# rogosprojects/klogs

Hardware: AMD Instinct MI355X
Metric: filtered log GB/s (whole node) at 1/2/4/8 MI355X; % of HBM peak (higher is better)
Workload: dtype u8

## Files before the change

### klogs_amd/csrc/klf_engine.cpp

```cpp
#include <hip/hip_runtime.h>

#include <unistd.h>

#include <algorithm>
#include <atomic>
#include <cerrno>
#include <chrono>
#include <condition_variable>
#include <cstdio>
#include <cstdlib>
#include <cstring>
#include <deque>
#include <memory>
#include <mutex>
#include <string>
#include <thread>
#include <vector>

#include "../../include/klf.h"
#include "../../include/klf_debug.h"
#include "klf_copypool.hpp"
#include "klf_fieldval.hpp"
#include "klf_groupkey.hpp"
#include "klf_kernels.hpp"
// ... 1265 lines not shown
  klf_engine* e = p.e;
  const klf_filter* f = p.f;
  const RunKnobs& k = p.k;
  const bool general = p.mode == klf::CompiledSet::kGeneral, none = p.mode == klf::CompiledSet::kNone;
  memset(static_cast<void*>(&a), 0, sizeof(a));
  a.bytes = p.d_bytes; a.segs = e->d_segs.as<SegDesc>(); a.nsegs = p.nsegs; a.ntiles = (uint32_t)p.ntiles;
  a.tile_seg = e->d_tile_seg.as<uint32_t>();
  a.build_tiles = (!p.same_layout && attempt == 0) ? 1u : 0u;
  a.tindex_wide = (p.ntiles > klf::kScanSmallTiles || k.tindex_wide) ? 1u : 0u;
  a.since_sec = f->since.sec; a.since_nsec = f->since.nsec; a.tail = f->tail;
  since_digits(f->since.sec, f->since.nsec, a.since_dig);
  a.grep_mode = (uint32_t)p.mode; a.match_all = e->cs.also_all ? 1u : 0u;
  a.lit = e->d_lit.as<uint8_t>(); a.lit_words = e->d_lit.as<uint32_t>(); a.lit_len = (uint32_t)e->cs.literal.size();
  a.lit_anchor = e->cs.literal_anchor;
  a.lit_anchor_byte = e->cs.literal.empty() ? 0u : e->cs.literal[e->cs.literal_anchor];
  memcpy(static_cast<void*>(&a.pats), &e->dpats, sizeof(a.pats));
  a.tstat = e->d_tstat.as<klf::TileStat>(); a.tile_base = e->d_tile_base.as<uint64_t>(); a.bsum = e->d_bsum.as<uint64_t>();
  a.slots = p.wave_pool ? nullptr : e->d_slots.as<uint32_t>(); a.wave_pool = p.wave_pool ? 1u : 0u;
  a.pool = e->d_pool.as<uint32_t>(); a.pool_cap = e->pool_cap; a.pool_chunk = s.pool_chunk;
  a.counters = e->d_counters.as<uint32_t>(); a.segout = segout_of(e);
  a.wpre = e->d_wpre.as<uint64_t>(); a.wgrp = a.wpre + p.nsegs + 1;
  a.out = e->d_out.as<uint8_t>(); a.out_cap = e->d_out.p ? e->d_out.cap : 0;
  a.stage_times = (f->flags & KLF_FILTER_STAGE_TIMES) && p.evs ? 1u : 0u;
  if (p.need_cand) { a.cand = e->d_cand.as<uint64_t>(); a.cand_cap = e->cand_cap; }
  if (p.need_hits) {
    a.qhits = e->d_qhits.as<uint64_t>(); a.qhits_cap = p.qhits_cap; a.hslots = e->d_hslots.as<uint16_t>();
    a.hflat = e->d_hflat.as<uint64_t>(); a.hflat_cap = p.hflat_cap;
  }
  a.trec = e->d_trec.as<klf::TRec>(); a.kbase = e->d_kbase.as<uint64_t>();
  a.truns = p.want_truns ? e->d_truns.as<uint32_t>() : nullptr;
// ... 1754 lines not shown
  std::vector<uint32_t> kinds;
  for (uint32_t i = 0; i < n; ++i) {
    ps.emplace_back(pats[i].bytes, pats[i].bytes + pats[i].len);
    kinds.push_back(pats[i].kind);
  }
  klf::CompiledSet cs;
  std::string err;
  int code = KLF_OK;
  if (!klf::compile_set(ps, kinds, cs, err, code)) return code;
  if (info) {
    info[0] = cs.qf_on ? 1u : 0u;
    info[1] = cs.qf_q;
    info[2] = cs.qf_stride;
    info[3] = cs.qf_needles;
    info[4] = cs.qf_anc_on ? 0x100u | cs.qf_anc_byte : 0u;
  }
  if (cs.mode != klf::CompiledSet::kGeneral || !cs.qf_on) return klf_debug_match(pats, n, content, len, match);
  *match = (cs.also_all || klf::prefilter_match(cs, content, len, phase)) ? 1 : 0;
  return KLF_OK;
}

extern "C" int klf_debug_prefilter_hits(const klf_pattern* pats, uint32_t n, const uint8_t* sample, size_t slen,
                                        const uint8_t* data, size_t dlen, uint64_t* out, char* layout, size_t cap) {
  if ((n && !pats) || (slen && !sample) || (dlen && !data) || !out) return KLF_EINVAL;
  std::vector<std::vector<uint8_t>> ps;
  std::vector<uint32_t> kinds;
  for (uint32_t i = 0; i < n; ++i) {
    ps.emplace_back(pats[i].bytes, pats[i].bytes + pats[i].len);
    kinds.push_back(pats[i].kind);
  }
// ... 5 lines not shown
  if (slen) {
    klf::DataStats st;
    klf::data_stats(sample, slen, cs.qf_fold, st);
    klf::place_needles(cs, &st);
  }
  const klf::PrefilterHits h = klf::prefilter_hits(cs, data, dlen);
  out[0] = cs.qf_stride;
  out[1] = cs.qf_q;
  out[2] = cs.qf_k;
  out[3] = cs.qf_anc_on ? 0x100u | cs.qf_anc_byte : 0u;
  out[4] = h.probes;
  out[5] = h.bitmap_hits;
  out[6] = h.anchor_hits;
  out[7] = h.verified;
  out[8] = h.pair_pass;
  if (layout && cap) { strncpy(layout, cs.qf_layout.c_str(), cap - 1); layout[cap - 1] = 0; }
  return KLF_OK;
}

extern "C" int klf_debug_compile(const klf_pattern* pats, uint32_t n, uint32_t* mode, char* err, size_t err_cap) {
  if ((n && !pats) || !mode) return KLF_EINVAL;
  std::vector<std::vector<uint8_t>> ps;
  std::vector<uint32_t> kinds;
  for (uint32_t i = 0; i < n; ++i) {
    ps.emplace_back(pats[i].bytes, pats[i].bytes + pats[i].len);
    kinds.push_back(pats[i].kind);
  }
  klf::CompiledSet cs;
  std::string e;
  int code = KLF_OK;
// ... 26 lines not shown
```

### klogs_amd/csrc/klf_kernels.hip

```cpp
#include <hip/hip_ext.h>
#include <hip/hip_runtime.h>

#include <cstdio>
#include <cstdlib>
#include <cstring>
#include <type_traits>

#include "klf_fieldval.hpp"
#include "klf_groupkey.hpp"
#include "klf_kernels.hpp"
#include "klf_ts.hpp"

namespace klf {
namespace {

#ifndef KLF_TIMELINE
#define KLF_TIMELINE 0
#endif
__device__ uint32_t g_abl_waves;
#if KLF_TIMELINE
__device__ uint64_t g_timeline[300000 * 8];
__device__ uint32_t g_lb_rounds, g_lb_spins;
#define KLF_STAMP(tile, k) do { if (threadIdx.x == 0 && (tile) < 300000) g_timeline[(size_t)(tile) * 8 + (k)] = __builtin_amdgcn_s_memtime(); } while (0)
#else
// ... 770 lines not shown
  if (MODE == kScanLit) {
    if (tl.dense) __threadfence_block();
    wave_lds_sync();
    lit_grep(list, tl.nlines, s_tile, s_lit, a, c, anc, pat, n);
  }
  if (tl.dense) __threadfence_block();
  wave_lds_sync();
}

constexpr uint32_t kNoHit = 0xFFFFFFFFu;
template <int QS, int QK, int QQ>
struct QProbe {
  static constexpr bool kMidIdx = QQ == 3 && QK == 2;
  static constexpr bool K3 = QK == 3 || QK == (int)kQfTwoLevel;
  static constexpr bool TWO = QK == (int)kQfTwoLevel;
  static_assert(!TWO || QS == 4, "the two-level probe runs at stride 4");
  static_assert(QQ == 3 || QQ == 4, "3- or 4-byte grams");
  const uint32_t* s_qf;
  const uint8_t* s_tile;
  uint32_t fold;
  struct Hash {
    uint32_t h, p, m, a;
  };
  __device__ __forceinline__ Hash hash(uint32_t g) const {
    const uint32_t gf = g | fold;
    const uint32_t f = K3 ? gf ^ bfe_u32(gf, 13, 11) : gf;
    Hash r;
    r.h = mul_u24(f, 0x9E3779u);
    if (QQ == 4) r.h = mad_u24(gf >> 8, 0x7F4A7Du, r.h);
    r.p = K3 ? mul_hi_u24(f, 0xC2B2AEu) : 0u;
    r.m = K3 ? mul_u24(f, 0x5BD1E9u) : 0u;
    r.a = TWO ? (((r.h >> 21) << 2) + kQfPairWords * 4u)
          : kMidIdx ? ((r.h >> 16) & ((kQfWords - 1u) << 2)) : ((r.h >> (32 - kQfBucketBits)) << 2);
    return r;
  }
  __device__ __forceinline__ uint32_t word(const Hash& r) const {
    return *reinterpret_cast<const uint32_t*>(reinterpret_cast<const uint8_t*>(s_qf) + r.a);
  }
  __device__ __forceinline__ static uint32_t test(uint32_t w, const Hash& r) {
    uint32_t t = K3 ? (w >> ((r.m >> 24) & 31u)) & (w >> (r.p & 31u))
                    : shr_byte1(w, r.h) & (w >> ((r.h >> 16) & 31u));
    if (K3) t &= w >> ((r.h >> 16) & 31u);
    if (TWO) t &= shr_byte1(w, r.m);
    return t;
  }
  __device__ __forceinline__ uint32_t hbits(uint32_t g) const {
    const Hash r = hash(g);
    return test(word(r), r);
  }
  template <class F>
  __device__ __forceinline__ void chunk_grams(const ScanTile& c, uint32_t ch, F&& f) const {
    const uint32_t o0 = c.my0 + 16u * ch;
    const uint4 x = *reinterpret_cast<const uint4*>(s_tile + o0);
    if constexpr (QS == 6) {
      f(x.x, 0);
      f(__builtin_amdgcn_alignbyte(x.z, x.y, 2u), 6);
      f(x.w, 12);
      return;
    }
    const uint32_t w4 = QS < 4 ? reinterpret_cast<const uint32_t*>(s_tile)[(o0 >> 2) + 4] : 0u;
    const uint32_t w[5] = {x.x, x.y, x.z, x.w, w4};
#pragma unroll
    for (int d = 0; d < 4; ++d)
// ... 69 lines not shown
      uint32_t w[2 * kPer];
#pragma unroll
      for (int k = 0; k < 2 * kPer; ++k) r[k] = hash(g[k]);
#pragma unroll
      for (int k = 0; k < 2 * kPer; ++k) w[k] = word(r[k]);
      uint32_t acc_a = 0, acc_b = 0;
#pragma unroll
      for (int k = 0; k < 2 * kPer; ++k) {
        const uint32_t t = test(w[k], r[k]);
        if (k < kPer) acc_a |= t; else acc_b |= t;
      }
      chit |= ((acc_a & 1u) << ca) | ((acc_b & 1u) << cb);
    }
    return chit;
  }
  __device__ __forceinline__ uint32_t fast_chunks(const ScanTile& c) const {
    const uint32_t rot = ((uint32_t)c.lane >> 1) & 7u;
    uint32_t chit = 0;
#pragma unroll
    for (int v = 0; v < (ABL(c, 4) ? 0 : 8); ++v) {
      const uint32_t ch = ((uint32_t)v + rot) & 7u;
      uint32_t acc = 0;
      chunk_grams(c, ch, [&](uint32_t g, int) __attribute__((always_inline)) { acc |= hbits(g); });
      chit |= (acc & 1u) << ch;
    }
    return chit;
  }
  __device__ __forceinline__ void positions(const ScanTile& c, uint32_t chit, uint32_t (&hq)[4]) const {
    for (uint32_t m = chit; m; m &= m - 1u) {
      const uint32_t ch = (uint32_t)__builtin_ctz(m);
      uint32_t hm = 0;
      chunk_grams(c, ch, [&](uint32_t g, int pos) __attribute__((always_inline)) { hm |= (hbits(g) & 1u) << pos; });
      or_quad(hq, ch >> 1, clip_chunk(c, hm, ch) << ((ch & 1u) * 16u));
    }
  }
  __device__ __forceinline__ void run(const ScanTile& c, uint32_t* s_list, uint32_t nlines, uint32_t (&hq)[4],
                                      uint32_t& xh) const {
    if constexpr (TWO) {
      two_level(c, s_list, nlines, hq, xh);
    } else {
      const uint32_t chit = (QS == 4 || QS == 6) ? fast_pairs(c) : fast_chunks(c);
      if (__any(chit != 0)) positions(c, chit, hq);
    }
  }
};
__device__ __forceinline__ void anchored_hits(const DevPatterns& P, const uint8_t* s_tile, const ScanTile& c, uint32_t anc,
                                              uint32_t pat, uint32_t afold, uint32_t (&hq)[4]) {
  const uint32_t* s32 = reinterpret_cast<const uint32_t*>(s_tile);
  const uint32_t npre = P.qf_anc_n, fold = P.qf_fold;
  for (uint32_t cm = anc; cm; cm &= cm - 1u) {
    const uint32_t ch = (uint32_t)__builtin_ctz(cm);
    const uint4 x = lane_chunk(s_tile, c, ch);
    uint32_t am = 0;
    for (uint32_t e = clip_chunk(c, eq_mask16(afold ? or4(x, afold) : x, pat), ch); e; e &= e - 1u) {
// ... 190 lines not shown

    LineCounts n;
    if (ABL(c, 128)) {
    } else if (!tl.dense) {
      line_work<MODE, FUSE>(s_list, a, c, ev, tl, s_tile, s_lit, any.anc, pat, fz, tile == range_t0, s_frun_all[FUSE ? wv : 0],
                            s_fmap_all[FUSE ? wv : 0], n);
    } else if (tl.pool_ok && !abl) {
      if (FUSE && lane == 0) a.counters[kCtrFuseBad] = 1u;
      line_work<MODE, FUSE>(a.pool + tl.pool_base, a, c, ev, tl, s_tile, s_lit, any.anc, pat, fz, tile == range_t0,
                            s_frun_all[FUSE ? wv : 0], s_fmap_all[FUSE ? wv : 0], n);
    }

    uint32_t tile_hits = 0;
    if constexpr (GEN) {
      uint32_t hq[4] = {0u, 0u, 0u, 0u}, xh = kNoHit;
      const QProbe<QS, QK, QQ> probe{s_qf, s_tile, a.pats.qf_fold};
      probe.run(c, s_list, tl.nlines, hq, xh);
      if (ANC && __any(any.anc != 0)) anchored_hits(a.pats, s_tile, c, any.anc, pat, afold, hq);
      if (ABL(c, 8)) {
        asm volatile("" ::"v"(hq[0] | hq[1] | hq[2] | hq[3] | xh));
        hq[0] = hq[1] = hq[2] = hq[3] = 0;
        xh = kNoHit;
      }
      if (__any((hq[0] | hq[1] | hq[2] | hq[3]) != 0u || xh != kNoHit) && (!abl || (KLF_ABL & (65536 | 131072))))
        tile_hits = emit_hits(a, c, hq, xh);
    }

    TileTotals tt;
    tt.pq = packed_counts(n, tl.nlines);
    tt.defer = __any(n.defer != 0);
    tt.hit = LIT && __any(n.hits != 0);
// ... 655 lines not shown
      uint4 E = Eb[0];
#pragma unroll
      for (int i = 1; i < kVerifyEnt; ++i)
        if (j == i) E = Eb[i];
      entry(E);
    }
  }
}

__device__ void verify_hit(const RunArgs& a, uint32_t tile, uint32_t s, int32_t p, const VerifyQ& vq) {
  const DevPatterns& P = a.pats;
  const SegDesc sd = a.segs[s];
  const int64_t rel_lo = (int64_t)(tile - sd.tile0) * kTile;
  const uint32_t gs = gword(a.bytes + sd.base + rel_lo + p);
  const uint32_t g = (gs | P.qf_fold) & P.qf_mask;
  const uint32_t b = qf_bucket(g, P.qf_w24, P.qf_k);
  verify_hit_from(a, tile, s, sd, p, gs, P.qf_head[b], P.qf_head[b + 1], vq);
}

constexpr int kVerifyBatch = 4;
struct VerifyLds {
  uint32_t qn[4];
  uint64_t qbuf[4][kVerifyQ][2];
};
__device__ __forceinline__ void verify_body(RunArgs& a, uint32_t bid, uint32_t nb, VerifyLds& L) {
  auto& s_qn = L.qn;
  auto& s_qbuf = L.qbuf;
  if (a.counters[2] || a.counters[kCtrHitsOver]) return;
  const int lane = threadIdx.x & 63, wv = threadIdx.x >> 6;
  if (lane == 0) s_qn[wv] = 0;
  wave_lds_sync();
// ... 13 lines not shown
      tile[u] = (uint32_t)hf;
      pp[u] = (int32_t)((hf >> 32) & 0xFFFFu);
      sg[u] = (uint32_t)(hf >> 48);
      if (sg[u] == 0xFFFFu) sg[u] = a.tile_seg[tile[u]];
    }
#pragma unroll
    for (int u = 0; u < kVerifyBatch; ++u) sd[u] = a.segs[sg[u]];
    uint32_t gg[kVerifyBatch];
#pragma unroll
    for (int u = 0; u < kVerifyBatch; ++u) {
      const int64_t rel_lo = (int64_t)(tile[u] - sd[u].tile0) * kTile;
      gg[u] = gword(a.bytes + sd[u].base + rel_lo + pp[u]);
    }
#pragma unroll
    for (int u = 0; u < kVerifyBatch; ++u) {
      const uint32_t b = qf_bucket((gg[u] | P.qf_fold) & P.qf_mask, P.qf_w24, P.qf_k);
      e0[u] = P.qf_head[b];
      e1[u] = P.qf_head[b + 1];
    }
    KLF_VSTAMP(1);
#pragma unroll
    for (int u = 0; u < kVerifyBatch; ++u)
      if (i0 + (uint32_t)u * stride < nf) {
#if KLF_ABL & 16
        if (pp[u] == 0x7FFF) atomicOr(&a.counters[13], sg[u]);
        continue;
#endif
        verify_hit_from(a, tile[u], sg[u], sd[u], pp[u], gg[u], e0[u], e1[u], vq);
      }
  }
  const uint32_t nh = a.counters[kCtrHits] < a.qhits_cap ? a.counters[kCtrHits] : a.qhits_cap;
// ... 3040 lines not shown
hipError_t launch_scan(const RunArgs& a, hipStream_t st, int num_cus) {
  const int occ = scan_occupancy<MODE, QS, QK, QQ, QA, FUSE>();
  uint32_t grid = (uint32_t)(num_cus * occ);
  if (grid > a.ntiles) grid = a.ntiles;
  if (FUSE) grid = (a.fuse_nranges + kThreads / 64 - 1) / (kThreads / 64);
  if (t_scan_ev[0])
    hipExtLaunchKernelGGL((k_scan<MODE, QS, QK, QQ, QA, FUSE>), dim3(grid), dim3(kThreads), 0, st, t_scan_ev[0],
                          t_scan_ev[1], 0, a, a.tile_seg, a.segs);
  else
    hipLaunchKernelGGL((k_scan<MODE, QS, QK, QQ, QA, FUSE>), dim3(grid), dim3(kThreads), 0, st, a, a.tile_seg,
                       a.segs);
  return hipGetLastError();
}
template <int QS, int QQ>
hipError_t launch_gen_q(const RunArgs& a, hipStream_t st, int num_cus) {
  if constexpr (QS == 4)
    if (a.pats.qf_k == kQfTwoLevel)
      return launch_scan<kScanGen, 4, (int)kQfTwoLevel, QQ>(a, st, num_cus);
  if constexpr (QS == 8)
    if (a.pats.qf_anc_on)
      return a.pats.qf_k == 2 ? launch_scan<kScanGen, QS, 2, QQ, true>(a, st, num_cus)
                              : launch_scan<kScanGen, QS, 3, QQ, true>(a, st, num_cus);
  if (a.pats.qf_anc_on) return hipErrorInvalidValue;
  return a.pats.qf_k == 2 ? launch_scan<kScanGen, QS, 2, QQ>(a, st, num_cus)
                          : launch_scan<kScanGen, QS, 3, QQ>(a, st, num_cus);
}
template <int QS>
hipError_t launch_gen(const RunArgs& a, hipStream_t st, int num_cus) {
  if constexpr (QS == 1)
    return a.pats.qf_w24 ? hipErrorInvalidValue : launch_gen_q<1, 3>(a, st, num_cus);
  else
    return a.pats.qf_w24 ? launch_gen_q<QS, 4>(a, st, num_cus) : launch_gen_q<QS, 3>(a, st, num_cus);
}
// ... 402 lines not shown
```

### klogs_amd/csrc/klf_kernels.hpp

```cpp
#pragma once
#include <hip/hip_runtime.h>
#include <stdint.h>

namespace klf {

constexpr int kThreads = 256;
constexpr int kLaneBytes = 128;
constexpr int kTile = 64 * kLaneBytes;
constexpr int kHalo = 64;
constexpr int kMaxFusedLiteral = 256;
constexpr uint64_t kSegAlign = 256;
constexpr uint64_t kAllocSlack = kTile + kHalo + 1024;
constexpr uint32_t kPlenEscape = 16383;
constexpr int kCompactLines = 1024;
constexpr uint32_t kNumCounters = 64;
constexpr uint32_t kCtrPool = 4;
constexpr uint32_t kMatchChunk = 8192;

constexpr int kSlots = kTile / 32 + 2;
constexpr uint32_t kScanSmallTiles = 1u << 20;
constexpr int kSlotStride = (kSlots + 3) & ~3;
constexpr int kRecHead = 4;
constexpr uint32_t kScanGroup = 8;
constexpr int kRecStride = (kRecHead + kSlots + 31) & ~31;
// ... 24 lines not shown
constexpr uint32_t kCtrTailDone = 18;
constexpr uint32_t kCtrPlanDone = 26;
constexpr uint32_t kCtrVerified = 10;
constexpr uint32_t kCtrDense = 14;
constexpr uint32_t kCtrFuseBad = 24;
constexpr uint32_t kCtrOutShort = 22;
constexpr uint32_t kCtrPairsOver = 15;
constexpr uint32_t kQfRegex = 1u << 24;
constexpr uint32_t kQfLoose = 1u << 25;
constexpr uint32_t kQfAnchored = 1u << 26;
constexpr size_t kNfaMaxLds = 64 * 1024;
constexpr uint32_t kCarryBias = 256;
constexpr uint32_t kRxPreNone = 0xFFFFFFFFu;
constexpr uint32_t kQfTwoLevel = 5;
constexpr uint32_t kQfPairWords = 2048;
__host__ __device__ inline uint32_t qf_pair_word(uint32_t p) { return (p >> 5) & (kQfPairWords - 1u); }
__host__ __device__ inline bool qf_k3(uint32_t k) { return k == 3 || k == kQfTwoLevel; }
__host__ __device__ inline uint32_t qf_f(uint32_t g, uint32_t k) {
  const uint32_t g24 = g & 0xFFFFFFu;
  return qf_k3(k) ? g24 ^ (g24 >> 13) : g24;
}
__host__ __device__ inline uint32_t qf_hash(uint32_t g, uint32_t w24, uint32_t k) {
  const uint32_t hi = w24 ? (g >> 8) & 0xFFFFFFu : 0u;
  return qf_f(g, k) * 0x9E3779u + hi * 0x7F4A7Du;
}
__host__ __device__ inline uint32_t qf_word(uint32_t h) { return h >> (32 - kQfBucketBits); }
__host__ __device__ inline uint32_t qf_bucket(uint32_t g, uint32_t w24, uint32_t k) {
  if (w24 == 0 && k == 2) return (qf_hash(g, w24, k) >> 18) & (kQfWords - 1u);
  if (k == kQfTwoLevel) return qf_hash(g, w24, k) >> 21;
  return qf_word(qf_hash(g, w24, k));
}
__host__ __device__ inline uint32_t qf_bloom_word(uint32_t g, uint32_t w24, uint32_t k) {
  return (k == kQfTwoLevel ? kQfPairWords : 0u) + qf_bucket(g, w24, k);
}
__host__ __device__ inline uint32_t qf_bits(uint32_t g, uint32_t h, uint32_t k) {
  const uint32_t f = qf_f(g, k);
  const uint32_t m = f * 0x5BD1E9u;
  if (!qf_k3(k)) return (1u << ((h >> 8) & 31u)) | (1u << ((h >> 16) & 31u));
  const uint32_t p = (uint32_t)(((uint64_t)f * 0xC2B2AEu) >> 32);
  const uint32_t b3 = (1u << ((m >> 24) & 31u)) | (1u << (p & 31u)) | (1u << ((h >> 16) & 31u));
  return k == kQfTwoLevel ? b3 | (1u << ((m >> 8) & 31u)) : b3;
}
__host__ __device__ inline bool qf_pass(const uint32_t* bm, uint32_t gq, uint32_t w24, uint32_t k) {
  if (k == kQfTwoLevel && !((bm[qf_pair_word(gq & 0xFFFFu)] >> (gq & 31u)) & 1u)) return false;
  const uint32_t h = qf_hash(gq, w24, k), bits = qf_bits(gq, h, k);
  return (bm[qf_bloom_word(gq, w24, k)] & bits) == bits;
}
constexpr uint32_t kGramHistPairs = 256;
constexpr uint32_t kGramHistWords = kGramHistPairs + 65536;
constexpr uint64_t kGramHistSample = 64u << 10;
constexpr uint32_t kQfK2MaxGrams = 1536;
__host__ __device__ inline bool qf_sampled(uint64_t p, uint32_t S) {
  if (S == 6) {
    const uint32_t r = (uint32_t)(p & 15u);
    return r == 0 || r == 6 || r == 12;
  }
  return p % S == 0;
}
// ... 78 lines not shown
  uint32_t nsegs;
  uint32_t ntiles;
  uint32_t* tile_seg;
  uint32_t build_tiles;
  uint32_t tindex_wide;
  int64_t since_sec;
  int32_t since_nsec;
  uint32_t since_dig[6];
  int64_t tail;
  uint32_t grep_mode;
  uint32_t match_all;
  const uint8_t* lit;
  uint32_t lit_len;
  uint32_t lit_anchor;
  uint32_t lit_anchor_byte;
  const uint32_t* lit_words;
  DevPatterns pats;
  TileStat* tstat;
  uint32_t* slots;
  uint32_t* pool;
  uint64_t pool_cap;
  uint32_t wave_pool;
  uint32_t pool_chunk;
  uint64_t* tile_base;
  uint64_t* bsum;
  uint64_t* mpart;
  uint64_t* csum;
  uint32_t* cmap;
  uint64_t cmap_cap;
  uint32_t* cseg;
// ... 239 lines not shown
```

### klogs_amd/csrc/klf_patterns.cpp

```cpp
#include "klf_patterns.hpp"

#include <algorithm>
#include <chrono>
#include <bitset>
#include <cstdio>
#include <cstdlib>
#include <cstring>
#include <map>
#include <set>
#include <unordered_map>
#include <queue>
#include <thread>

#include "../../include/klf.h"
#include "klf_kernels.hpp"

namespace klf {
namespace {

using ByteSet = std::bitset<256>;

ByteSet range_set(int lo, int hi) {
  ByteSet s;
  if (hi < lo) return s;
// ... 1351 lines not shown
  }
  size_t cap = 64;
  uint32_t shift = 26;
  while (cap < 2 * grams.size()) cap <<= 1, --shift;
  std::vector<uint32_t> seen(cap, ~0u);
  double hit_share = 0;
  for (uint32_t g : grams) {
    uint32_t i = (g * 0x9E3779B1u) >> shift;
    while (seen[i] != ~0u && seen[i] != g) i = (i + 1) & (uint32_t)(cap - 1);
    if (seen[i] == g) continue;
    seen[i] = g;
    hit_share += gram_share(st, g, c.qf_q);
  }
  const double samples = qf_samples_per_tile(c.qf_stride);
  double hits = samples * std::min(1.0, hit_share);
  const double per_probe = c.qf_k == kQfTwoLevel ? 6.0 + (c.qf_q == 4 ? 1.0 : 0.0)
                                                 : 7.0 + (c.qf_q == 4 ? 3.0 : 0.0) + (c.qf_k == 3 ? 6.5 : 0.0);
  double cost = per_probe * samples / 64.0;
  if (c.qf_anc_on) {
    cost += 60.0;
    double pass = 0;
    for (size_t j = 0; j + 1 < c.qf_anc_pre.size(); j += 2)
      pass += c.qf_anc_pre[j + 1] == ~0u ? gram_share(st, c.qf_anc_pre[j], 4)
                                         : gram_share(st, c.qf_anc_pre[j] & 0xFFFFFFu, 3);
    hits += 8192.0 * std::min(1.0, pass);
  }
  return cost + 40.0 * hits;
}

void place_tables(CompiledSet& out, const DataStats* st);

}

void place_needles(CompiledSet& out, const DataStats* st) {
  std::vector<uint32_t> ac_next, ac_dict;
  std::vector<uint8_t> ac_accept;
  std::vector<int32_t> ac_out;
  std::vector<uint64_t> rx_b, rx_follow;
  std::vector<CompiledSet::NeedleSet> variants;
  std::vector<int32_t> user_map;
  ac_next.swap(out.ac_next);
  ac_dict.swap(out.ac_dict);
  ac_accept.swap(out.ac_accept);
  ac_out.swap(out.ac_out);
  rx_b.swap(out.rx_b);
  rx_follow.swap(out.rx_follow);
  variants.swap(out.qf_variants);
  user_map.swap(out.user_map);
  CompiledSet best;
  double best_cost = 0;
  bool have = false;
  std::vector<std::string> seen;
  for (uint32_t v = 0; v < variants.size(); ++v)
    for (int cand = 0; cand < 4; ++cand) {
      const int anchored = cand & 1;
      const uint32_t qmax = cand < 2 ? 4u : 3u;
      if (qmax == 3 && !(st && st->nbytes)) continue;
      if (const char* qv = getenv("KLF_QF_QMAX"))
        if (st && st->nbytes && (uint32_t)atoi(qv) != qmax) continue;
      CompiledSet c = out;
      const auto& ns = variants[v];
      c.qf_variant = v;
      c.qf_needle = ns.s;
      c.qf_nflags = ns.flags;
      c.qf_nrx = ns.rx;
      c.qf_needles = (uint32_t)ns.s.size();
      c.rx_pre = ns.rx_pre;
      choose_layout(c, st, anchored != 0, qmax);
      if (anchored && !c.qf_anc_on) continue;
      {
        const std::string key = std::to_string(v) + "/" + c.qf_layout;
        if (std::find(seen.begin(), seen.end(), key) != seen.end()) continue;
        seen.push_back(key);
      }
      const auto t0 = std::chrono::steady_clock::now();
      place_tables(c, st);
      const auto t1 = std::chrono::steady_clock::now();
      double cost;
      if (st && st->nbytes) {
        cost = layout_cost(c, *st);
      } else {
        cost = 1e6 * qf_samples_per_tile(c.qf_stride) / 8192.0 + (c.qf_anc_on ? c.qf_anc_share * 1e3 : 0.0);
      }
      char buf[64];
      snprintf(buf, sizeof buf, " k=%u [est %.0f VALU/tile]", c.qf_k, cost);
      c.qf_layout += buf;
      if (getenv("KLF_DIAG"))
        fprintf(stderr, "[klf] layout candidate (variant %u): %s (tables %.0f us, cost %.0f us)\n", v, c.qf_layout.c_str(),
                std::chrono::duration<double, std::micro>(t1 - t0).count(),
                std::chrono::duration<double, std::micro>(std::chrono::steady_clock::now() - t1).count());
      if (!have || cost < best_cost) {
        best = std::move(c);
        best_cost = cost;
        have = true;
      }
    }
  if (have) out = std::move(best);
  out.qf_variants.swap(variants);
  out.user_map.swap(user_map);
  out.ac_next.swap(ac_next);
  out.ac_dict.swap(ac_dict);
  out.ac_accept.swap(ac_accept);
  out.ac_out.swap(ac_out);
  out.rx_b.swap(rx_b);
  out.rx_follow.swap(rx_follow);
}

namespace {

void place_tables(CompiledSet& out, const DataStats* st) {
  const uint32_t q = out.qf_q, S = out.qf_stride;
  const bool hist = st && st->pair.size() >= 65536 && st->pair_tot > 0;
  const double nsample = st && st->nbytes ? (double)st->nbytes : 1.0;
  static const double pair_w = getenv("KLF_QF_PAIRW") ? atof(getenv("KLF_QF_PAIRW")) : 0.05;
  const bool loose = out.qf_fold != 0;
  out.qf_bitmap.assign(kQfWords, 0u);
  out.qf_head.clear();
  out.qf_ent.clear();
  out.qf_nbytes.clear();
  auto gram_at = [&](const std::string& s, uint32_t k) {
    uint32_t g = 0;
    for (uint32_t b = 0; b < q; ++b) g |= (uint32_t)(uint8_t)s[k + b] << (8 * b);
    return (g | out.qf_fold) & out.qf_mask;
  };
  uint8_t rank[256];
// ... 24 lines not shown
    uint32_t get(uint32_t g) const { return cnt[slot(g)]; }
    void add(uint32_t g) {
      const uint32_t i = slot(g);
      key[i] = g;
      ++cnt[i];
    }
  } used(out.qf_needle.size() * S + 1);
  std::vector<uint64_t> gcost;
  std::vector<std::pair<uint32_t, uint32_t>> bent;
  bent.reserve(out.qf_needle.size() * S);
  const size_t n = out.qf_needle.size();
  size_t nprobed = 0;
  for (size_t i = 0; i < n; ++i) nprobed += out.qf_nshort[i] ? 0 : 1;
  const char* two = getenv("KLF_QF_TWO");
  const bool two_ok = S == 4 && !out.qf_anc_on && !(two && !strcmp(two, "0"));
  out.qf_k = (two_ok && two && !strcmp(two, "force")) ? kQfTwoLevel
             : nprobed * S <= kQfK2MaxGrams ? 2u : two_ok ? kQfTwoLevel : 3u;
  const uint32_t w24 = q == 4 ? 24u : 0u;
  for (uint32_t i = 0; i < n; ++i) {
    const std::string& s = out.qf_needle[i];
    if (out.qf_nshort[i]) {
      const uint32_t k = out.qf_nanc[i], g = gram_at(s, k);
      bent.push_back({qf_bucket(g, w24, out.qf_k), i << 8 | k});
      continue;
    }
    const uint32_t amax = (uint32_t)std::min<size_t>(s.size() - (q + S - 1), 255 - (S - 1));
    gcost.resize(amax + S);
    for (uint32_t k = 0; k < amax + S; ++k) {
      const uint32_t g = gram_at(s, k);
      const uint64_t u = used.get(g);
      uint64_t c;
      if (hist) {
// ... 5 lines not shown
        c = 2 * u;
        for (uint32_t b = 0; b < q; ++b) c += common((uint8_t)s[k + b]);
      }
      gcost[k] = c;
    }
    uint32_t best_a = 0;
    uint64_t best = UINT64_MAX;
    for (uint32_t a = 0; a <= amax; ++a) {
      uint64_t sc = 0;
      for (uint32_t j = 0; j < S; ++j) sc = hist ? sc + gcost[a + j] : std::max(sc, gcost[a + j]);
      if (sc < best) { best = sc; best_a = a; }
    }
    for (uint32_t j = 0; j < S; ++j) {
      const uint32_t k = best_a + j, g = gram_at(s, k);
      used.add(g);
      const uint32_t h = qf_hash(g, w24, out.qf_k);
      const uint32_t bw = qf_bucket(g, w24, out.qf_k);
      out.qf_bitmap[qf_bloom_word(g, w24, out.qf_k)] |= qf_bits(g, h, out.qf_k);
      if (out.qf_k == kQfTwoLevel) {
        const uint32_t g16 = g & 0xFFFFu, fv = out.qf_fold & 0xFFFFu & g16;
        for (uint32_t x = fv;; x = (x - 1u) & fv) {
          const uint32_t pr = g16 & ~x;
          out.qf_bitmap[qf_pair_word(pr)] |= 1u << (pr & 31u);
          if (!x) break;
        }
      }
      bent.push_back({bw, i << 8 | k});
    }
  }
  std::vector<uint32_t> noff;
  for (auto& ns : out.qf_needle) {
    noff.push_back((uint32_t)out.qf_nbytes.size());
    for (size_t b = 0; b < ns.size(); b += 4) {
      uint32_t w = 0;
      for (size_t j = 0; j < 4 && b + j < ns.size(); ++j) w |= (uint32_t)(uint8_t)ns[b + j] << (8 * j);
      out.qf_nbytes.push_back(w);
    }
  }
  out.qf_head.assign(kQfWords + 1, 0u);
  for (auto& be : bent) out.qf_head[be.first + 1]++;
  for (uint32_t b = 0; b < kQfWords; ++b) out.qf_head[b + 1] += out.qf_head[b];
  out.qf_ent.assign((size_t)bent.size() * 4, 0u);
  std::vector<uint32_t> fill(out.qf_head.begin(), out.qf_head.end() - 1);
  for (auto& be : bent) {
    const uint32_t v = be.second, i = v >> 8;
    uint32_t* en = &out.qf_ent[(size_t)fill[be.first]++ * 4];
    en[0] = noff[i];
    en[1] = (uint32_t)out.qf_needle[i].size() | (v & 0xFFu) << 16 | out.qf_nflags[i] |
            (out.qf_nshort[i] ? kQfAnchored : 0u);
    en[2] = out.qf_nrx[i];
    {
      const auto& nd = out.qf_needle[i];
      const uint32_t k = v & 0xFFu;
      uint32_t w = 0;
      for (uint32_t j = 0; j < 4 && k + j < nd.size(); ++j) w |= (uint32_t)(uint8_t)nd[k + j] << (8 * j);
      en[3] = w;
    }
  }
}

}

void stats_finish(DataStats& st) {
  st.marg.assign(256, 0.0);
  st.inv_marg.assign(256, 0.0);
  st.pair_tot = 0;
  st.inv_tot = 0;
  if (st.pair.size() >= 65536) {
    for (uint32_t x = 0; x < 65536; ++x) st.marg[x & 0xFFu] += st.pair[x];
    for (double m : st.marg) st.pair_tot += m;
    if (st.pair_tot > 0) {
      st.inv_tot = 1.0 / st.pair_tot;
      for (int c = 0; c < 256; ++c) st.inv_marg[c] = st.pair_tot / (st.marg[c] + 128.0);
// ... 27 lines not shown
    st.pair[g >> 16] += 2;
  }
  stats_finish(st);
}

PrefilterHits prefilter_hits(const CompiledSet& cs, const uint8_t* s, size_t n) {
  PrefilterHits r;
  const uint32_t S = cs.qf_stride, w24 = cs.qf_q == 4 ? 24u : 0u;
  for (size_t p = 0; p < n; ++p) {
    uint32_t g = 0;
    for (uint32_t b = 0; b < 4; ++b) g |= (uint32_t)(p + b < n ? s[p + b] : 0) << (8 * b);
    bool hit = false;
    if (qf_sampled(p, S)) {
      ++r.probes;
      const uint32_t gq = (g | cs.qf_fold) & cs.qf_mask;
      hit = qf_pass(cs.qf_bitmap.data(), gq, w24, cs.qf_k);
      r.bitmap_hits += hit;
      if (cs.qf_k == kQfTwoLevel) r.pair_pass += (cs.qf_bitmap[qf_pair_word(gq & 0xFFFFu)] >> (gq & 31u)) & 1u;
    }
    if (!hit && cs.qf_anc_on && ((uint32_t)s[p] | (cs.qf_anc_fold & 0xFFu)) == cs.qf_anc_byte) {
      for (size_t j = 0; j + 1 < cs.qf_anc_pre.size() && !hit; j += 2)
        hit = ((g | cs.qf_fold) & cs.qf_anc_pre[j + 1]) == cs.qf_anc_pre[j];
      r.anchor_hits += hit;
    }
    if (!hit) continue;
    const uint32_t b = qf_bucket((g | cs.qf_fold) & cs.qf_mask, w24, cs.qf_k);
    for (uint32_t e = cs.qf_head[b]; e < cs.qf_head[b + 1]; ++e) {
      const uint32_t* E = cs.qf_ent.data() + 4 * (size_t)e;
      const uint32_t m = E[1] & 0xFFFFu, k = (E[1] >> 16) & 0xFFu;
      const int64_t x = (int64_t)p - (int64_t)k;
      if (x < 0 || (uint64_t)x + m > n) continue;
      const uint8_t* nb = reinterpret_cast<const uint8_t*>(cs.qf_nbytes.data() + E[0]);
      const uint8_t lm = (E[1] & kQfLoose) ? 0x20 : 0;
      bool eq = true;
      for (uint32_t j = 0; j < m && eq; ++j) eq = (uint8_t)(s[x + j] | lm) == nb[j];
      r.verified += eq;
    }
  }
  return r;
}

// ... 9 lines not shown
    for (uint64_t m = c; m; m &= m - 1) nd |= cs.rx_follow[(size_t)r * 64 + __builtin_ctzll(m)];
    d = nd;
    if (!d) return false;
  }
  return (d & cs.rx_end[r]) != 0;
}

bool prefilter_match(const CompiledSet& cs, const uint8_t* s, size_t n, uint32_t phase) {
  const uint32_t S = cs.qf_stride;
  for (size_t p = 0; p < n; ++p) {
    uint32_t g = 0;
    for (uint32_t b = 0; b < 4; ++b) g |= (uint32_t)(p + b < n ? s[p + b] : 0) << (8 * b);
    bool hit = false;
    if (qf_sampled(p + 16 - phase % 16, S)) {
      const uint32_t gq = (g | cs.qf_fold) & cs.qf_mask;
      hit = qf_pass(cs.qf_bitmap.data(), gq, cs.qf_q == 4 ? 24u : 0u, cs.qf_k);
    }
    if (!hit && cs.qf_anc_on && ((uint32_t)s[p] | (cs.qf_anc_fold & 0xFFu)) == cs.qf_anc_byte)
      for (size_t j = 0; j + 1 < cs.qf_anc_pre.size() && !hit; j += 2)
        hit = ((g | cs.qf_fold) & cs.qf_anc_pre[j + 1]) == cs.qf_anc_pre[j];
    if (!hit) continue;
    g = (g | cs.qf_fold) & cs.qf_mask;
    const uint32_t b = qf_bucket(g, cs.qf_q == 4 ? 24u : 0u, cs.qf_k);
    for (uint32_t e = cs.qf_head[b]; e < cs.qf_head[b + 1]; ++e) {
      const uint32_t* E = cs.qf_ent.data() + 4 * (size_t)e;
      const uint32_t m = E[1] & 0xFFFFu, k = (E[1] >> 16) & 0xFFu;
      const int64_t x = (int64_t)p - (int64_t)k;
      if (x < 0 || (uint64_t)x + m > n) continue;
      const uint8_t* nb = reinterpret_cast<const uint8_t*>(cs.qf_nbytes.data() + E[0]);
      const uint8_t lm = (E[1] & kQfLoose) ? 0x20 : 0;
      bool eq = true;
      for (uint32_t j = 0; j < m && eq; ++j) eq = (uint8_t)(s[x + j] | lm) == nb[j];
      if (!eq) continue;
      if (!(E[1] & kQfRegex)) return true;
      if ((cs.rx_flags[E[2]] & 1u) || nfa_window(cs, E[2], s, n, (size_t)x)) return true;
    }
  }
  return false;
// ... 4 lines not shown
```

### klogs_amd/csrc/klf_patterns.hpp

```cpp
#pragma once
#include <stdint.h>
#include <stddef.h>

#include <array>
#include <string>
#include <vector>

namespace klf {

constexpr int kMaxRegexPositions = 64;
constexpr int kMaxRegexes = 1024;

struct GlushkovTables {
  std::vector<uint64_t> follow;
  uint64_t first = 0;
  uint64_t last = 0;
  uint64_t init0 = 0;
  uint64_t end_accept = 0;
  bool accept_at_start = false;
  bool accept_empty = false;
  std::vector<std::vector<uint8_t>> pos_bytes;
  std::vector<std::array<uint64_t, 4>> pos_bits;
  int npos = 0;
};
// ... 40 lines not shown
  uint32_t rx_classes = 0;
  std::vector<uint8_t> rx_class;
  std::vector<uint64_t> rx_b;
  std::vector<uint64_t> rx_follow;
  std::vector<uint64_t> rx_first, rx_last, rx_init0, rx_end;
  std::vector<uint32_t> rx_flags;
  std::vector<uint32_t> rx_pre;
  uint32_t rx_maxpos = 0;

  bool qf_on = false;
  uint32_t qf_q = 4;
  uint32_t qf_stride = 1;
  uint32_t qf_fold = 0;
  uint32_t qf_mask = ~0u;
  uint32_t qf_k = 3;
  std::vector<uint32_t> qf_bitmap;
  std::vector<uint32_t> qf_head;
  std::vector<uint32_t> qf_ent;
  std::vector<uint32_t> qf_nbytes;
  uint32_t qf_needles = 0;
  std::vector<std::string> qf_needle;
  std::vector<uint32_t> qf_nflags, qf_nrx;
  bool qf_tuned = false;
  std::string qf_why;
  bool qf_anc_on = false;
  uint32_t qf_anc_byte = 0;
  uint32_t qf_anc_fold = 0;
  double qf_anc_share = 0;
  std::vector<uint32_t> qf_anc_pre;
  std::vector<uint8_t> qf_nshort;
// ... 54 lines not shown
```

### klogs_amd/engine.py

```python
from __future__ import annotations

import ctypes as C
import os
from dataclasses import dataclass
from pathlib import Path
from typing import Iterable, List, Optional, Sequence, Tuple

import numpy as np

_LIB_DIR = Path(os.environ.get("KLF_LIB_DIR", Path(__file__).resolve().parent / "_lib"))
_LIB_PATH = _LIB_DIR / "libklf.so"

KLF_OK = 0
KLF_EINVAL = -1
KLF_ENOMEM = -2
KLF_EHIP = -3
KLF_EPATTERN = -4
KLF_ETOOBIG = -5
KLF_ESTATE = -6
KLF_EIO = -7
KLF_PAT_LITERAL = 0
KLF_PAT_REGEX = 1
GO_ZERO_TIME = (-62135596800, 0)
TIME_MIN_SEC = -(1 << 63)
# ... 266 lines not shown
    rc = _lib.klf_debug_compile(arr, n, C.byref(mode), err, 512)
    return rc, MODE_NAMES.get(mode.value, "?"), err.value.decode()


def debug_match(content: bytes, grep=(), match=()) -> bool:
    arr, n, keep = _patterns(grep, match)
    m = C.c_int()
    buf = C.create_string_buffer(content, len(content) or 1)
    _check(_lib.klf_debug_match(arr, n, buf, len(content), C.byref(m)))
    return bool(m.value)


def debug_prefilter(content: bytes, grep=(), match=(), phase: int = 0):
    arr, n, keep = _patterns(grep, match)
    m = C.c_int()
    info = (C.c_uint32 * 5)()
    buf = C.create_string_buffer(content, len(content) or 1)
    _check(_lib.klf_debug_prefilter(arr, n, buf, len(content), phase, C.byref(m), info))
    return bool(m.value), dict(on=bool(info[0]), q=info[1], stride=info[2], needles=info[3],
                               anchor=(info[4] & 0xFF) if info[4] else None)


def debug_prefilter_hits(sample: bytes, data: bytes, grep=(), match=()):
    arr, n, keep = _patterns(grep, match)
    out = (C.c_uint64 * 9)()
    lay = C.create_string_buffer(256)
    sb = C.create_string_buffer(sample, len(sample) or 1)
    db = C.create_string_buffer(data, len(data) or 1)
    _check(_lib.klf_debug_prefilter_hits(arr, n, sb, len(sample), db, len(data), out, lay, 256))
    return dict(stride=out[0], q=out[1], k=out[2], anchor=(out[3] & 0xFF) if out[3] else None, probes=out[4],
                bitmap_hits=out[5], anchor_hits=out[6], verified=out[7], pair_pass=out[8],
                layout=lay.value.decode())


def debug_factors(pattern: bytes, want: int = 0):
    buf = C.create_string_buffer(4096)
    n, pre, loose = C.c_uint32(), C.c_uint32(), C.c_uint32()
    p = C.create_string_buffer(pattern, len(pattern) or 1)
    rc = _lib.klf_debug_factors(p, len(pattern), want, buf, 4096, C.byref(n), C.byref(pre), C.byref(loose))
    if rc == KLF_EINVAL:
        return None
    _check(rc)
    alts = buf.raw.split(b"\0")[: n.value]
    return alts, (None if pre.value == 0xFFFFFFFF else pre.value), bool(loose.value)


# ... 444 lines not shown
```

Measured before the change: 5701.

## Add exact perfect-hash gram prefilter for small stride-4 needle sets

Adds a new prefilter mode (k=6) for small stride-4, unanchored needle sets. Grams are placed into a collision-free multiplicative-hash table that stores the full gram, so each probe is one LDS load and one compare instead of a Bloom test over several hash bits. The intent is fewer VALU operations per probe and fewer false-positive hits reaching verification. The layout chooser costs this candidate and selects it when sample stats are present. It adds host-side search for a collision-free multiplier and a new kernel instantiation, and falls back when more than 192 distinct grams exist or no multiplier is found.

After: 5861 (median of 6 runs). 1.03x the previous value.

```diff
diff --git a/klogs_amd/csrc/klf_engine.cpp b/klogs_amd/csrc/klf_engine.cpp
--- a/klogs_amd/csrc/klf_engine.cpp
+++ b/klogs_amd/csrc/klf_engine.cpp
@@ -1303,6 +1303,7 @@
   a.lit = e->d_lit.as<uint8_t>(); a.lit_words = e->d_lit.as<uint32_t>(); a.lit_len = (uint32_t)e->cs.literal.size();
   a.lit_anchor = e->cs.literal_anchor;
   a.lit_anchor_byte = e->cs.literal.empty() ? 0u : e->cs.literal[e->cs.literal_anchor];
+  a.qf_mul = e->cs.qf_mul;
   memcpy(static_cast<void*>(&a.pats), &e->dpats, sizeof(a.pats));
   a.tstat = e->d_tstat.as<klf::TileStat>(); a.tile_base = e->d_tile_base.as<uint64_t>(); a.bsum = e->d_bsum.as<uint64_t>();
   a.slots = p.wave_pool ? nullptr : e->d_slots.as<uint32_t>(); a.wave_pool = p.wave_pool ? 1u : 0u;
@@ -3087,6 +3088,8 @@
     info[2] = cs.qf_stride;
     info[3] = cs.qf_needles;
     info[4] = cs.qf_anc_on ? 0x100u | cs.qf_anc_byte : 0u;
+    info[5] = cs.qf_k;
+    info[6] = cs.qf_mul;
   }
   if (cs.mode != klf::CompiledSet::kGeneral || !cs.qf_on) return klf_debug_match(pats, n, content, len, match);
   *match = (cs.also_all || klf::prefilter_match(cs, content, len, phase)) ? 1 : 0;
@@ -3122,6 +3125,8 @@
   out[6] = h.anchor_hits;
   out[7] = h.verified;
   out[8] = h.pair_pass;
+  out[9] = cs.qf_grams;
+  out[10] = cs.qf_mul;
   if (layout && cap) { strncpy(layout, cs.qf_layout.c_str(), cap - 1); layout[cap - 1] = 0; }
   return KLF_OK;
 }
diff --git a/klogs_amd/csrc/klf_kernels.hip b/klogs_amd/csrc/klf_kernels.hip
--- a/klogs_amd/csrc/klf_kernels.hip
+++ b/klogs_amd/csrc/klf_kernels.hip
@@ -808,11 +808,14 @@
   static constexpr bool kMidIdx = QQ == 3 && QK == 2;
   static constexpr bool K3 = QK == 3 || QK == (int)kQfTwoLevel;
   static constexpr bool TWO = QK == (int)kQfTwoLevel;
+  static constexpr bool EX = QK == (int)kQfExact;
   static_assert(!TWO || QS == 4, "the two-level probe runs at stride 4");
+  static_assert(!EX || QS == 4, "the exact probe runs at stride 4");
   static_assert(QQ == 3 || QQ == 4, "3- or 4-byte grams");
   const uint32_t* s_qf;
   const uint8_t* s_tile;
   uint32_t fold;
+  uint32_t mul;
   struct Hash {
     uint32_t h, p, m, a;
   };
@@ -838,9 +841,19 @@
     if (TWO) t &= shr_byte1(w, r.m);
     return t;
   }
+  __device__ __forceinline__ uint32_t ex_sample(uint32_t g) const { return g | fold; }
+  __device__ __forceinline__ uint32_t ex_word(uint32_t gf) const {
+    const uint32_t a = (mul_u24(gf, mul) >> 16) & ((kQfWords - 1u) << 2);
+    return *reinterpret_cast<const uint32_t*>(reinterpret_cast<const uint8_t*>(s_qf) + a);
+  }
   __device__ __forceinline__ uint32_t hbits(uint32_t g) const {
-    const Hash r = hash(g);
-    return test(word(r), r);
+    if constexpr (EX) {
+      const uint32_t gf = ex_sample(g);
+      return ex_word(gf) == gf ? 1u : 0u;
+    } else {
+      const Hash r = hash(g);
+      return test(word(r), r);
+    }
   }
   template <class F>
   __device__ __forceinline__ void chunk_grams(const ScanTile& c, uint32_t ch, F&& f) const {
@@ -940,6 +953,24 @@
     }
     return chit;
   }
+  __device__ __forceinline__ uint64_t fast_exact(const ScanTile& c) const {
+    const uint32_t rot = ((uint32_t)c.lane >> 1) & 7u;
+    uint64_t lanes = 0;
+#pragma unroll
+    for (int v = 0; v < (ABL(c, 4) ? 0 : 8); v += 2) {
+      const uint4 xa = lane_chunk(s_tile, c, ((uint32_t)v + rot) & 7u);
+      const uint4 xb = lane_chunk(s_tile, c, ((uint32_t)v + 1u + rot) & 7u);
+      const uint32_t g[8] = {xa.x, xa.y, xa.z, xa.w, xb.x, xb.y, xb.z, xb.w};
+      uint32_t gf[8], w[8];
+#pragma unroll
+      for (int k = 0; k < 8; ++k) gf[k] = ex_sample(g[k]);
+#pragma unroll
+      for (int k = 0; k < 8; ++k) w[k] = ex_word(gf[k]);
+#pragma unroll
+      for (int k = 0; k < 8; ++k) lanes |= __ballot(w[k] == gf[k]);
+    }
+    return lanes;
+  }
   __device__ __forceinline__ uint32_t fast_chunks(const ScanTile& c) const {
     const uint32_t rot = ((uint32_t)c.lane >> 1) & 7u;
     uint32_t chit = 0;
@@ -964,6 +995,9 @@
                                       uint32_t& xh) const {
     if constexpr (TWO) {
       two_level(c, s_list, nlines, hq, xh);
+    } else if constexpr (EX) {
+      const uint64_t lanes = fast_exact(c);
+      if (lanes) positions(c, ((lanes >> c.lane) & 1u) ? 0xFFu : 0u, hq);
     } else {
       const uint32_t chit = (QS == 4 || QS == 6) ? fast_pairs(c) : fast_chunks(c);
       if (__any(chit != 0)) positions(c, chit, hq);
@@ -1184,7 +1218,9 @@
     uint32_t tile_hits = 0;
     if constexpr (GEN) {
       uint32_t hq[4] = {0u, 0u, 0u, 0u}, xh = kNoHit;
-      const QProbe<QS, QK, QQ> probe{s_qf, s_tile, a.pats.qf_fold};
+      constexpr bool EX = QK == (int)kQfExact;
+      const QProbe<QS, QK, QQ> probe{s_qf, s_tile, a.pats.qf_fold | ((EX && QQ == 3) ? 0xFF000000u : 0u),
+                                     EX ? a.qf_mul : 0u};
       probe.run(c, s_list, tl.nlines, hq, xh);
       if (ANC && __any(any.anc != 0)) anchored_hits(a.pats, s_tile, c, any.anc, pat, afold, hq);
       if (ABL(c, 8)) {
@@ -1870,7 +1906,7 @@
   const int64_t rel_lo = (int64_t)(tile - sd.tile0) * kTile;
   const uint32_t gs = gword(a.bytes + sd.base + rel_lo + p);
   const uint32_t g = (gs | P.qf_fold) & P.qf_mask;
-  const uint32_t b = qf_bucket(g, P.qf_w24, P.qf_k);
+  const uint32_t b = qf_bucket(g, P.qf_w24, P.qf_k, a.qf_mul);
   verify_hit_from(a, tile, s, sd, p, gs, P.qf_head[b], P.qf_head[b + 1], vq);
 }
 
@@ -1914,7 +1950,7 @@
     }
 #pragma unroll
     for (int u = 0; u < kVerifyBatch; ++u) {
-      const uint32_t b = qf_bucket((gg[u] | P.qf_fold) & P.qf_mask, P.qf_w24, P.qf_k);
+      const uint32_t b = qf_bucket((gg[u] | P.qf_fold) & P.qf_mask, P.qf_w24, P.qf_k, a.qf_mul);
       e0[u] = P.qf_head[b];
       e1[u] = P.qf_head[b + 1];
     }
@@ -4985,9 +5021,13 @@
 }
 template <int QS, int QQ>
 hipError_t launch_gen_q(const RunArgs& a, hipStream_t st, int num_cus) {
-  if constexpr (QS == 4)
+  if constexpr (QS == 4) {
     if (a.pats.qf_k == kQfTwoLevel)
       return launch_scan<kScanGen, 4, (int)kQfTwoLevel, QQ>(a, st, num_cus);
+    if (a.pats.qf_k == kQfExact && !a.pats.qf_anc_on)
+      return launch_scan<kScanGen, 4, (int)kQfExact, QQ>(a, st, num_cus);
+  }
+  if (a.pats.qf_k == kQfExact) return hipErrorInvalidValue;
   if constexpr (QS == 8)
     if (a.pats.qf_anc_on)
       return a.pats.qf_k == 2 ? launch_scan<kScanGen, QS, 2, QQ, true>(a, st, num_cus)
diff --git a/klogs_amd/csrc/klf_kernels.hpp b/klogs_amd/csrc/klf_kernels.hpp
--- a/klogs_amd/csrc/klf_kernels.hpp
+++ b/klogs_amd/csrc/klf_kernels.hpp
@@ -62,6 +62,13 @@
 constexpr uint32_t kRxPreNone = 0xFFFFFFFFu;
 constexpr uint32_t kQfTwoLevel = 5;
 constexpr uint32_t kQfPairWords = 2048;
+constexpr uint32_t kQfExact = 6;
+constexpr uint32_t kQfExactMaxGrams = 192;
+constexpr uint32_t kQfExactTries = 512;
+__host__ __device__ inline uint32_t qf_exact_slot(uint32_t g, uint32_t mul) {
+  return (((g & 0xFFFFFFu) * mul) >> 18) & (kQfWords - 1u);
+}
+__host__ __device__ inline uint32_t qf_exact_word(uint32_t g, uint32_t w24) { return w24 ? g : g | 0xFF000000u; }
 __host__ __device__ inline uint32_t qf_pair_word(uint32_t p) { return (p >> 5) & (kQfPairWords - 1u); }
 __host__ __device__ inline bool qf_k3(uint32_t k) { return k == 3 || k == kQfTwoLevel; }
 __host__ __device__ inline uint32_t qf_f(uint32_t g, uint32_t k) {
@@ -73,7 +80,8 @@
   return qf_f(g, k) * 0x9E3779u + hi * 0x7F4A7Du;
 }
 __host__ __device__ inline uint32_t qf_word(uint32_t h) { return h >> (32 - kQfBucketBits); }
-__host__ __device__ inline uint32_t qf_bucket(uint32_t g, uint32_t w24, uint32_t k) {
+__host__ __device__ inline uint32_t qf_bucket(uint32_t g, uint32_t w24, uint32_t k, uint32_t mul = 0u) {
+  if (k == kQfExact) return qf_exact_slot(g, mul);
   if (w24 == 0 && k == 2) return (qf_hash(g, w24, k) >> 18) & (kQfWords - 1u);
   if (k == kQfTwoLevel) return qf_hash(g, w24, k) >> 21;
   return qf_word(qf_hash(g, w24, k));
@@ -89,7 +97,8 @@
   const uint32_t b3 = (1u << ((m >> 24) & 31u)) | (1u << (p & 31u)) | (1u << ((h >> 16) & 31u));
   return k == kQfTwoLevel ? b3 | (1u << ((m >> 8) & 31u)) : b3;
 }
-__host__ __device__ inline bool qf_pass(const uint32_t* bm, uint32_t gq, uint32_t w24, uint32_t k) {
+__host__ __device__ inline bool qf_pass(const uint32_t* bm, uint32_t gq, uint32_t w24, uint32_t k, uint32_t mul = 0u) {
+  if (k == kQfExact) return bm[qf_exact_slot(gq, mul)] == qf_exact_word(gq, w24);
   if (k == kQfTwoLevel && !((bm[qf_pair_word(gq & 0xFFFFu)] >> (gq & 31u)) & 1u)) return false;
   const uint32_t h = qf_hash(gq, w24, k), bits = qf_bits(gq, h, k);
   return (bm[qf_bloom_word(gq, w24, k)] & bits) == bits;
@@ -198,6 +207,7 @@
   uint32_t lit_len;
   uint32_t lit_anchor;
   uint32_t lit_anchor_byte;
+  uint32_t qf_mul;
   const uint32_t* lit_words;
   DevPatterns pats;
   TileStat* tstat;
diff --git a/klogs_amd/csrc/klf_patterns.cpp b/klogs_amd/csrc/klf_patterns.cpp
--- a/klogs_amd/csrc/klf_patterns.cpp
+++ b/klogs_amd/csrc/klf_patterns.cpp
@@ -1389,8 +1389,9 @@
   }
   const double samples = qf_samples_per_tile(c.qf_stride);
   double hits = samples * std::min(1.0, hit_share);
-  const double per_probe = c.qf_k == kQfTwoLevel ? 6.0 + (c.qf_q == 4 ? 1.0 : 0.0)
-                                                 : 7.0 + (c.qf_q == 4 ? 3.0 : 0.0) + (c.qf_k == 3 ? 6.5 : 0.0);
+  const double per_probe = c.qf_k == kQfExact      ? 4.0
+                           : c.qf_k == kQfTwoLevel ? 6.0 + (c.qf_q == 4 ? 1.0 : 0.0)
+                                                   : 7.0 + (c.qf_q == 4 ? 3.0 : 0.0) + (c.qf_k == 3 ? 6.5 : 0.0);
   double cost = per_probe * samples / 64.0;
   if (c.qf_anc_on) {
     cost += 60.0;
@@ -1403,7 +1404,12 @@
   return cost + 40.0 * hits;
 }
 
-void place_tables(CompiledSet& out, const DataStats* st);
+bool place_tables(CompiledSet& out, const DataStats* st, bool exact = false);
+
+int exact_knob() {
+  const char* v = getenv("KLF_QF_EXACT");
+  return !v ? 1 : !strcmp(v, "0") ? 0 : !strcmp(v, "force") ? 2 : 1;
+}
 
 }
 
@@ -1425,11 +1431,16 @@
   CompiledSet best;
   double best_cost = 0;
   bool have = false;
+  const char* two = getenv("KLF_QF_TWO");
+  const int xknob = (two && !strcmp(two, "force") && exact_knob() == 1) ? 0 : exact_knob();
+  const bool tuned = st && st->nbytes;
   std::vector<std::string> seen;
   for (uint32_t v = 0; v < variants.size(); ++v)
-    for (int cand = 0; cand < 4; ++cand) {
+    for (int cand = 0; cand < 8; ++cand) {
       const int anchored = cand & 1;
-      const uint32_t qmax = cand < 2 ? 4u : 3u;
+      const bool exact = cand >= 4;
+      if (exact && (anchored || xknob == 0 || !(tuned || xknob == 2))) continue;
+      const uint32_t qmax = (cand & 2) ? 3u : 4u;
       if (qmax == 3 && !(st && st->nbytes)) continue;
       if (const char* qv = getenv("KLF_QF_QMAX"))
         if (st && st->nbytes && (uint32_t)atoi(qv) != qmax) continue;
@@ -1443,23 +1454,34 @@
       c.rx_pre = ns.rx_pre;
       choose_layout(c, st, anchored != 0, qmax);
       if (anchored && !c.qf_anc_on) continue;
+      if (exact && (c.qf_stride != 4 || c.qf_anc_on)) continue;
       {
-        const std::string key = std::to_string(v) + "/" + c.qf_layout;
+        const std::string key = std::to_string(v) + "/" + c.qf_layout + (exact ? "/exact" : "");
         if (std::find(seen.begin(), seen.end(), key) != seen.end()) continue;
         seen.push_back(key);
       }
       const auto t0 = std::chrono::steady_clock::now();
-      place_tables(c, st);
+      const bool placed = place_tables(c, st, exact);
       const auto t1 = std::chrono::steady_clock::now();
+      if (!placed) {
+        if (getenv("KLF_DIAG"))
+          fprintf(stderr, "[klf] layout candidate (variant %u): %s k=%u: %u grams not placed (%.0f us)\n", v,
+                  c.qf_layout.c_str(), kQfExact, c.qf_grams, std::chrono::duration<double, std::micro>(t1 - t0).count());
+        continue;
+      }
       double cost;
       if (st && st->nbytes) {
         cost = layout_cost(c, *st);
       } else {
         cost = 1e6 * qf_samples_per_tile(c.qf_stride) / 8192.0 + (c.qf_anc_on ? c.qf_anc_share * 1e3 : 0.0);
       }
-      char buf[64];
-      snprintf(buf, sizeof buf, " k=%u [est %.0f VALU/tile]", c.qf_k, cost);
+      char buf[96];
+      if (exact)
+        snprintf(buf, sizeof buf, " k=%u [est %.0f VALU/tile] mul=0x%06x grams=%u", c.qf_k, cost, c.qf_mul, c.qf_grams);
+      else
+        snprintf(buf, sizeof buf, " k=%u [est %.0f VALU/tile]", c.qf_k, cost);
       c.qf_layout += buf;
+      if (exact && xknob == 2) cost -= 1e12;
       if (getenv("KLF_DIAG"))
         fprintf(stderr, "[klf] layout candidate (variant %u): %s (tables %.0f us, cost %.0f us)\n", v, c.qf_layout.c_str(),
                 std::chrono::duration<double, std::micro>(t1 - t0).count(),
@@ -1483,7 +1505,7 @@
 
 namespace {
 
-void place_tables(CompiledSet& out, const DataStats* st) {
+bool place_tables(CompiledSet& out, const DataStats* st, bool exact) {
   const uint32_t q = out.qf_q, S = out.qf_stride;
   const bool hist = st && st->pair.size() >= 65536 && st->pair_tot > 0;
   const double nsample = st && st->nbytes ? (double)st->nbytes : 1.0;
@@ -1538,8 +1560,13 @@
   for (size_t i = 0; i < n; ++i) nprobed += out.qf_nshort[i] ? 0 : 1;
   const char* two = getenv("KLF_QF_TWO");
   const bool two_ok = S == 4 && !out.qf_anc_on && !(two && !strcmp(two, "0"));
-  out.qf_k = (two_ok && two && !strcmp(two, "force")) ? kQfTwoLevel
+  out.qf_k = exact ? kQfExact
+             : (two_ok && two && !strcmp(two, "force")) ? kQfTwoLevel
              : nprobed * S <= kQfK2MaxGrams ? 2u : two_ok ? kQfTwoLevel : 3u;
+  out.qf_mul = 0;
+  out.qf_grams = 0;
+  if (exact && (S != 4 || out.qf_anc_on)) return false;
+  std::vector<uint32_t> egram;
   const uint32_t w24 = q == 4 ? 24u : 0u;
   for (uint32_t i = 0; i < n; ++i) {
     const std::string& s = out.qf_needle[i];
@@ -1575,6 +1602,11 @@
     for (uint32_t j = 0; j < S; ++j) {
       const uint32_t k = best_a + j, g = gram_at(s, k);
       used.add(g);
+      if (exact) {
+        egram.push_back(g);
+        bent.push_back({0u, i << 8 | k});
+        continue;
+      }
       const uint32_t h = qf_hash(g, w24, out.qf_k);
       const uint32_t bw = qf_bucket(g, w24, out.qf_k);
       out.qf_bitmap[qf_bloom_word(g, w24, out.qf_k)] |= qf_bits(g, h, out.qf_k);
@@ -1588,6 +1620,36 @@
       }
       bent.push_back({bw, i << 8 | k});
     }
+  }
+  for (uint32_t x : used.cnt) out.qf_grams += x ? 1u : 0u;
+  if (exact) {
+    std::vector<uint32_t> dg = egram;
+    std::sort(dg.begin(), dg.end());
+    dg.erase(std::unique(dg.begin(), dg.end()), dg.end());
+    if (dg.size() > kQfExactMaxGrams) return false;
+    for (size_t j = 1; j < dg.size(); ++j)
+      if ((dg[j] & 0xFFFFFFu) == (dg[j - 1] & 0xFFFFFFu)) return false;
+    std::vector<uint32_t> owner(kQfWords, 0u);
+    uint32_t mul = 0x9E3779u, found = 0;
+    for (uint32_t t = 1; t <= kQfExactTries && !found; ++t) {
+      bool ok = true;
+      for (size_t j = 0; j < dg.size() && ok; ++j) {
+        uint32_t& o = owner[qf_exact_slot(dg[j], mul)];
+        ok = o != t;
+        o = t;
+      }
+      if (ok) found = mul;
+      else mul = ((mul * 0x343FDu + 0x269EC3u) & 0xFFFFFFu) | 1u;
+    }
+    if (!found) return false;
+    out.qf_mul = found;
+    for (uint32_t s = 0; s < kQfWords; ++s) {
+      uint32_t e = 0;
+      while (qf_exact_slot(e, found) == s) ++e;
+      out.qf_bitmap[s] = e;
+    }
+    for (uint32_t g : dg) out.qf_bitmap[qf_exact_slot(g, found)] = qf_exact_word(g, w24);
+    for (size_t j = 0; j < bent.size(); ++j) bent[j].first = qf_exact_slot(egram[j], found);
   }
   std::vector<uint32_t> noff;
   for (auto& ns : out.qf_needle) {
@@ -1618,6 +1680,7 @@
       en[3] = w;
     }
   }
+  return true;
 }
 
 }
@@ -1675,7 +1738,7 @@
     if (qf_sampled(p, S)) {
       ++r.probes;
       const uint32_t gq = (g | cs.qf_fold) & cs.qf_mask;
-      hit = qf_pass(cs.qf_bitmap.data(), gq, w24, cs.qf_k);
+      hit = qf_pass(cs.qf_bitmap.data(), gq, w24, cs.qf_k, cs.qf_mul);
       r.bitmap_hits += hit;
       if (cs.qf_k == kQfTwoLevel) r.pair_pass += (cs.qf_bitmap[qf_pair_word(gq & 0xFFFFu)] >> (gq & 31u)) & 1u;
     }
@@ -1685,7 +1748,7 @@
       r.anchor_hits += hit;
     }
     if (!hit) continue;
-    const uint32_t b = qf_bucket((g | cs.qf_fold) & cs.qf_mask, w24, cs.qf_k);
+    const uint32_t b = qf_bucket((g | cs.qf_fold) & cs.qf_mask, w24, cs.qf_k, cs.qf_mul);
     for (uint32_t e = cs.qf_head[b]; e < cs.qf_head[b + 1]; ++e) {
       const uint32_t* E = cs.qf_ent.data() + 4 * (size_t)e;
       const uint32_t m = E[1] & 0xFFFFu, k = (E[1] >> 16) & 0xFFu;
@@ -1725,14 +1788,14 @@
     bool hit = false;
     if (qf_sampled(p + 16 - phase % 16, S)) {
       const uint32_t gq = (g | cs.qf_fold) & cs.qf_mask;
-      hit = qf_pass(cs.qf_bitmap.data(), gq, cs.qf_q == 4 ? 24u : 0u, cs.qf_k);
+      hit = qf_pass(cs.qf_bitmap.data(), gq, cs.qf_q == 4 ? 24u : 0u, cs.qf_k, cs.qf_mul);
     }
     if (!hit && cs.qf_anc_on && ((uint32_t)s[p] | (cs.qf_anc_fold & 0xFFu)) == cs.qf_anc_byte)
       for (size_t j = 0; j + 1 < cs.qf_anc_pre.size() && !hit; j += 2)
         hit = ((g | cs.qf_fold) & cs.qf_anc_pre[j + 1]) == cs.qf_anc_pre[j];
     if (!hit) continue;
     g = (g | cs.qf_fold) & cs.qf_mask;
-    const uint32_t b = qf_bucket(g, cs.qf_q == 4 ? 24u : 0u, cs.qf_k);
+    const uint32_t b = qf_bucket(g, cs.qf_q == 4 ? 24u : 0u, cs.qf_k, cs.qf_mul);
     for (uint32_t e = cs.qf_head[b]; e < cs.qf_head[b + 1]; ++e) {
       const uint32_t* E = cs.qf_ent.data() + 4 * (size_t)e;
       const uint32_t m = E[1] & 0xFFFFu, k = (E[1] >> 16) & 0xFFu;
diff --git a/klogs_amd/csrc/klf_patterns.hpp b/klogs_amd/csrc/klf_patterns.hpp
--- a/klogs_amd/csrc/klf_patterns.hpp
+++ b/klogs_amd/csrc/klf_patterns.hpp
@@ -78,6 +78,8 @@
   uint32_t qf_fold = 0;
   uint32_t qf_mask = ~0u;
   uint32_t qf_k = 3;
+  uint32_t qf_mul = 0;
+  uint32_t qf_grams = 0;
   std::vector<uint32_t> qf_bitmap;
   std::vector<uint32_t> qf_head;
   std::vector<uint32_t> qf_ent;
diff --git a/klogs_amd/engine.py b/klogs_amd/engine.py
--- a/klogs_amd/engine.py
+++ b/klogs_amd/engine.py
@@ -304,22 +304,22 @@
 def debug_prefilter(content: bytes, grep=(), match=(), phase: int = 0):
     arr, n, keep = _patterns(grep, match)
     m = C.c_int()
-    info = (C.c_uint32 * 5)()
+    info = (C.c_uint32 * 7)()
     buf = C.create_string_buffer(content, len(content) or 1)
     _check(_lib.klf_debug_prefilter(arr, n, buf, len(content), phase, C.byref(m), info))
     return bool(m.value), dict(on=bool(info[0]), q=info[1], stride=info[2], needles=info[3],
-                               anchor=(info[4] & 0xFF) if info[4] else None)
+                               anchor=(info[4] & 0xFF) if info[4] else None, k=info[5], mul=info[6])
 
 
 def debug_prefilter_hits(sample: bytes, data: bytes, grep=(), match=()):
     arr, n, keep = _patterns(grep, match)
-    out = (C.c_uint64 * 9)()
+    out = (C.c_uint64 * 11)()
     lay = C.create_string_buffer(256)
     sb = C.create_string_buffer(sample, len(sample) or 1)
     db = C.create_string_buffer(data, len(data) or 1)
     _check(_lib.klf_debug_prefilter_hits(arr, n, sb, len(sample), db, len(data), out, lay, 256))
     return dict(stride=out[0], q=out[1], k=out[2], anchor=(out[3] & 0xFF) if out[3] else None, probes=out[4],
-                bitmap_hits=out[5], anchor_hits=out[6], verified=out[7], pair_pass=out[8],
+                bitmap_hits=out[5], anchor_hits=out[6], verified=out[7], pair_pass=out[8], grams=out[9], mul=out[10],
                 layout=lay.value.decode())
 
 
```
